# minaskar/tempest

Measured on AMD Instinct MI355X. Metric: particle-mutation-steps/s (whole job), 10-D Rosenbrock, higher is better.
Workload: dtype f64; 1 GPU; rosenbrock10d_n1048576 (BASELINE config 4: 10-D Rosenbrock, 1048576 particles sharded over 1 GPU(s), 1048576 per GPU); n_dim=10, particles_per_gpu=1048576, particles_global=1048576, sample=tpcn, resample=mult, clustering=False, n_total=4194304, step=one PS iteration, callbacks=torch-ROCm tensor callbacks (the drop-in contract: prior20, rosenbrock_torch)

## Files before the change

include/tempest_hip.h:

```cpp
#ifndef TEMPEST_HIP_H
#define TEMPEST_HIP_H

#include <stdint.h>

#ifdef __cplusplus
extern "C" {
#endif

typedef struct tph_ctx tph_ctx;

#define TPH_VERSION 100

#define TPH_KERNEL_TPCN 0
#define TPH_KERNEL_RWM 1

#define TPH_BC_STRICT 0
#define TPH_BC_PERIODIC 1
#define TPH_BC_REFLECTIVE 2

#define TPH_KEY_U 0
#define TPH_KEY_X 1
#define TPH_KEY_LOGL 2
#define TPH_KEY_LOGMIX 3

// ... 27 lines not shown
#define TPH_OPT_MF_DEAL 19
#define TPH_OPT_BLK_STAGE 20
#define TPH_OPT_GMM_KERNEL 21
#define TPH_OPT_FORMS_MFMA 22
int tph_set_option(tph_ctx* ctx, int option, int value);

typedef int (*tph_allreduce_fn)(void* user, int64_t offset, int64_t count, int dtype, int op);
typedef int (*tph_allgather_fn)(void* user, int64_t send_offset, int64_t recv_offset, int64_t count, int dtype);
int tph_comm_attach(tph_ctx* ctx, int rank, int world, void* buf_dev, int64_t buf_bytes, tph_allreduce_fn allreduce,
                    tph_allgather_fn allgather, void* user);
int tph_comm_detach(tph_ctx* ctx);
#define TPH_P2P_HANDLE_BYTES 64
int tph_comm_p2p_export(tph_ctx* ctx, void* handle_out );
int tph_comm_p2p_attach(tph_ctx* ctx, const void* handles , int* ok_out);
int tph_comm_p2p_active(const tph_ctx* ctx);
int tph_comm_p2p_status(tph_ctx* ctx);
int tph_comm_stats(tph_ctx* ctx, int64_t* out , int reset);
int tph_comm_allreduce_dev(tph_ctx* ctx, void* data_dev, int64_t count, int dtype, int op);

int tph_history_append(tph_ctx* ctx, const double* u_dev, const double* x_dev, const double* logl_dev,
                       int64_t n, int64_t ld, double beta, double logz, int64_t n_global);
int64_t tph_history_size(const tph_ctx* ctx);
int tph_history_iterations(const tph_ctx* ctx);
int tph_history_clear(tph_ctx* ctx);
int tph_history_memory(tph_ctx* ctx, int64_t* out9_host);
int tph_history_read(tph_ctx* ctx, int key, int64_t off, int64_t n, double* out_host);
int tph_history_ptr(tph_ctx* ctx, int key, void** dev_ptr, int64_t* ld);
int tph_history_load(tph_ctx* ctx, const double* u_host, const double* x_host, const double* logl_host,
                     int64_t n, int T, const double* beta_t, const double* logz_t, const int64_t* n_t_local,
                     const int64_t* n_t_global);

int tph_reweight_partials(tph_ctx* ctx, const double* betas_host, int nb, double* out_dev );
int tph_reweight_eval(tph_ctx* ctx, const double* betas_host, int nb, double* out_host );
int tph_weights(tph_ctx* ctx, double beta, double vmax, double s1, double* w_dev);
int tph_logw(tph_ctx* ctx, double beta, int64_t n_h_global, double* logw_dev);

int tph_trim_threshold_global(tph_ctx* ctx, const double* w_dev, int64_t n, double ess, int bins,
                              double* out_dev , double* out_host );
int tph_cdf_global(tph_ctx* ctx, const double* w_dev, int64_t n, const double* thr_dev , double* cdf_dev,
                   double* total_host );
int tph_resample_select_global(tph_ctx* ctx, const double* cdf_dev, int64_t n, int64_t n_slots, int scheme, uint64_t seed,
                               uint32_t tick, uint32_t tag, double u0, double pscale, int64_t* idx_dev);
int tph_resample_put_global(tph_ctx* ctx, const int64_t* idx_dev , int64_t n_slots, int64_t n_local,
                            double* u_out, double* x_out, double* logl_out, int64_t ld_out);
int tph_multinomial_counts_global(tph_ctx* ctx, const double* cdf_dev, int64_t n, const double* kept_count_dev, int factor,
                                  int64_t n_draw_max, uint64_t seed, uint32_t tick, uint32_t tag, int32_t* counts_dev);
int tph_fit_modes_global(tph_ctx* ctx, const int32_t* counts_dev, const int32_t* labels_dev, int64_t n, int K,
                         double* means_dev, double* covs_dev, double* chol_dev, double* inv_dev, double* cholinv_dev );

int tph_sum_sq_max(tph_ctx* ctx, const double* w_dev, int64_t n, double* out_host );

int tph_trim_threshold(tph_ctx* ctx, const double* w_dev, int64_t n, double ess, int bins,
                       double* out_dev , double* out_host );

int tph_cdf(tph_ctx* ctx, const double* w_dev, int64_t n, const double* thr_dev , double* cdf_dev);
int tph_resample_systematic(tph_ctx* ctx, const double* cdf_dev, int64_t n, int64_t n_out, int64_t i0,
                            int64_t size_global, double u0, double renorm, int64_t* idx_dev);
int tph_resample_multinomial(tph_ctx* ctx, const double* cdf_dev, int64_t n, int64_t n_out, uint64_t seed,
                             uint32_t tick, uint32_t tag, int64_t item0, int64_t* idx_dev);
int tph_resample_select(tph_ctx* ctx, const double* cdf_dev, int64_t n, int64_t n_slots, int scheme, uint64_t seed,
                        uint32_t tick, uint32_t tag, double u0, double w_before, double w_upto, double w_total,
                        int is_last, int64_t* idx_dev);
int tph_gather(tph_ctx* ctx, const int64_t* idx_dev, int64_t n_out, double* u_out, double* x_out,
               double* logl_out, int64_t ld_out);
int tph_posterior_rows(tph_ctx* ctx, int key, const int64_t* idx_dev, int64_t m, const double* w_dev, double wdiv,
                       double* x_out , double* logl_out , double* w_out );
// ... 91 lines not shown
```

tempest_amd/_lib.py:

```python
import ctypes as C
import os

_HERE = os.path.dirname(os.path.abspath(__file__))
LIB_PATH = os.path.join(_HERE, "csrc", "libtempest_hip.so")

c_i64 = C.c_int64
c_u64 = C.c_uint64
c_u32 = C.c_uint32
c_dbl = C.c_double
c_int = C.c_int
ptr = C.c_void_p

SIGNATURES = {
    "tph_last_error": (C.c_char_p, []),
    "tph_version": (c_int, []),
    "tph_ctx_create": (c_int, [c_int, c_int, c_i64, ptr, C.POINTER(ptr)]),
    "tph_ctx_destroy": (c_int, [ptr]),
    "tph_set_stream": (c_int, [ptr, ptr]),
    "tph_synchronize": (c_int, [ptr]),
    "tph_warmup": (c_int, [ptr]),
    "tph_set_option": (c_int, [ptr, c_int, c_int]),
    "tph_history_append": (c_int, [ptr, ptr, ptr, ptr, c_i64, c_i64, c_dbl, c_dbl, c_i64]),
    "tph_history_size": (c_i64, [ptr]),
    "tph_history_iterations": (c_int, [ptr]),
    "tph_history_clear": (c_int, [ptr]),
    "tph_history_memory": (c_int, [ptr, ptr]),
    "tph_history_read": (c_int, [ptr, c_int, c_i64, c_i64, ptr]),
    "tph_history_ptr": (c_int, [ptr, c_int, C.POINTER(ptr), C.POINTER(c_i64)]),
    "tph_history_load": (c_int, [ptr, ptr, ptr, ptr, c_i64, c_int, ptr, ptr, ptr, ptr]),
    "tph_reweight_partials": (c_int, [ptr, ptr, c_int, ptr]),
    "tph_reweight_eval": (c_int, [ptr, ptr, c_int, ptr]),
    "tph_bench_reweight_time": (c_int, [ptr, c_dbl, c_int, c_int, ptr]),
    "tph_bench_membw_time": (c_int, [ptr, c_int, c_i64, c_int, ptr]),
    "tph_bench_fp64_time": (c_int, [ptr, c_int, ptr]),
    "tph_student_sums": (c_int, [ptr, ptr, ptr, ptr, c_int, c_i64, ptr, c_int, ptr]),
    "tph_student_weights": (c_int, [ptr, ptr, ptr, ptr, c_int, c_i64, c_dbl, ptr]),
    "tph_bench_mf_normals": (c_int, [ptr, c_u64, c_u64, c_u64, c_int, ptr]),
    "tph_bench_mf_counters": (c_int, [ptr, ptr]),
    "tph_weights": (c_int, [ptr, c_dbl, c_dbl, c_dbl, ptr]),
    "tph_logw": (c_int, [ptr, c_dbl, c_i64, ptr]),
    "tph_sum_sq_max": (c_int, [ptr, ptr, c_i64, ptr]),
    "tph_trim_threshold": (c_int, [ptr, ptr, c_i64, c_dbl, c_int, ptr, ptr]),
    "tph_cdf": (c_int, [ptr, ptr, c_i64, ptr, ptr]),
    "tph_resample_systematic": (c_int, [ptr, ptr, c_i64, c_i64, c_i64, c_i64, c_dbl, c_dbl, ptr]),
    "tph_resample_multinomial": (c_int, [ptr, ptr, c_i64, c_i64, c_u64, c_u32, c_u32, c_i64, ptr]),
    "tph_resample_select": (c_int, [ptr, ptr, c_i64, c_i64, c_int, c_u64, c_u32, c_u32, c_dbl, c_dbl, c_dbl, c_dbl, c_int, ptr]),
    "tph_gather": (c_int, [ptr, ptr, c_i64, ptr, ptr, ptr, c_i64]),
    "tph_multinomial_counts": (c_int, [ptr, ptr, c_i64, ptr, c_int, c_i64, c_u64, c_u32, c_u32, ptr]),
    "tph_prior_draw": (c_int, [ptr, ptr, c_i64, c_i64, c_u64, c_u32, c_i64]),
    "tph_inf_repair": (c_int, [ptr, ptr, ptr, ptr, c_i64, c_i64, c_u64, c_u32, c_i64, ptr]),
    "tph_inf_repair_src": (c_int, [ptr, ptr, ptr, ptr, c_i64, c_i64, c_u64, c_u32, c_i64, ptr, ptr]),
    "tph_propose": (c_int, [ptr, c_int, ptr, ptr, c_i64, c_i64, c_int, ptr, ptr, ptr, ptr, ptr, ptr,
                            c_u64, c_u32, c_i64, ptr, ptr, ptr, ptr, ptr]),
    "tph_accept": (c_int, [ptr, c_int, c_dbl, ptr, ptr, ptr, ptr, ptr, ptr, ptr, ptr, ptr, c_i64, c_i64,
                           c_int, ptr, c_u64, c_u32, c_i64, ptr, ptr, ptr, ptr]),
    "tph_adapt": (c_int, [ptr, c_int, ptr, ptr, c_int, c_dbl, c_int, c_int, c_int, ptr, ptr, ptr, c_int, ptr, c_i64]),
    "tph_accept_sums_global": (c_int, [ptr, ptr, c_i64, c_int, ptr, c_int]),
    "tph_posterior_rows": (c_int, [ptr, c_int, ptr, c_i64, ptr, c_dbl, ptr, ptr, ptr]),
    "tph_marginals_layout": (c_i64, [c_int]),
    "tph_marginals_scratch_words": (c_i64, [c_i64, c_int, c_int, c_int, c_int, c_int]),
    "tph_marginals": (c_int, [ptr, ptr, c_i64, c_int, ptr, ptr, c_int, ptr, c_int, c_int, ptr, c_int, ptr, ptr, c_i64,
                              ptr, ptr, ptr, ptr, ptr, ptr, ptr, ptr]),
    "tph_index_compose": (c_int, [ptr, ptr, ptr, c_i64, ptr]),
    "tph_cluster_counts": (c_int, [ptr, ptr, c_i64, c_int, ptr]),
# ... 2 lines not shown
    "tph_weighted_moments": (c_int, [ptr, ptr, c_i64, ptr]),
    "tph_weighted_sums": (c_int, [ptr, ptr, c_i64, ptr]),
    "tph_weighted_cov_centered": (c_int, [ptr, ptr, c_i64, ptr, ptr]),
    "tph_weighted_moments_shifted": (c_int, [ptr, ptr, c_i64, ptr, ptr]),
    "tph_compact_indices": (c_int, [ptr, ptr, c_i64, ptr, ptr]),
    "tph_gather_u_affine": (c_int, [ptr, ptr, c_i64, ptr, ptr, ptr, ptr, c_i64, ptr]),
    "tph_affine": (c_int, [ptr, ptr, c_i64, c_i64, ptr, ptr]),
    "tph_x_weighted_sums": (c_int, [ptr, ptr, c_i64, c_i64, ptr, ptr, ptr]),
    "tph_x_weighted_cov": (c_int, [ptr, ptr, c_i64, c_i64, ptr, ptr, ptr]),
    "tph_gmm_estep": (c_int, [ptr, ptr, c_i64, c_i64, ptr, ptr, c_int, c_int, ptr, c_int, c_dbl, ptr, ptr, ptr, ptr, ptr]),
    "tph_gmm_em_state_doubles": (c_i64, [c_int, c_int]),
    "tph_gmm_em_begin": (c_int, [ptr, ptr, c_i64, c_i64, c_int, ptr, ptr]),
    "tph_gmm_em_run": (c_int, [ptr, ptr, c_i64, c_i64, ptr, ptr, c_int, c_int, ptr, ptr, c_dbl, c_dbl, c_int, c_int]),
    "tph_cv_sum": (c_int, [ptr, ptr, c_i64, ptr, ptr, ptr]),
    "tph_volume_variation": (c_int, [ptr, ptr, c_i64, ptr, ptr]),
    "tph_comm_attach": (c_int, [ptr, c_int, c_int, ptr, c_i64, ptr, ptr, ptr]),
    "tph_comm_detach": (c_int, [ptr]),
    "tph_comm_p2p_export": (c_int, [ptr, ptr]),
    "tph_comm_p2p_attach": (c_int, [ptr, ptr, ptr]),
    "tph_comm_p2p_active": (c_int, [ptr]),
    "tph_comm_p2p_status": (c_int, [ptr]),
    "tph_comm_stats": (c_int, [ptr, ptr, c_int]),
    "tph_comm_allreduce_dev": (c_int, [ptr, ptr, c_i64, c_int, c_int]),
    "tph_resample_put_global": (c_int, [ptr, ptr, c_i64, c_i64, ptr, ptr, ptr, c_i64]),
    "tph_trim_threshold_global": (c_int, [ptr, ptr, c_i64, c_dbl, c_int, ptr, ptr]),
    "tph_cdf_global": (c_int, [ptr, ptr, c_i64, ptr, ptr, ptr]),
    "tph_resample_select_global": (c_int, [ptr, ptr, c_i64, c_i64, c_int, c_u64, c_u32, c_u32, c_dbl, c_dbl, ptr]),
    "tph_multinomial_counts_global": (c_int, [ptr, ptr, c_i64, ptr, c_int, c_i64, c_u64, c_u32, c_u32, ptr]),
    "tph_fit_modes_global": (c_int, [ptr, ptr, ptr, c_i64, c_int, ptr, ptr, ptr, ptr, ptr]),
}

ALLREDUCE_FN = C.CFUNCTYPE(c_int, ptr, c_i64, c_i64, c_int, c_int)
ALLGATHER_FN = C.CFUNCTYPE(c_int, ptr, c_i64, c_i64, c_i64, c_int)


class TempestHipError(RuntimeError):
    pass


_lib = None


def load(path=None):
    global _lib
    if _lib is not None and path is None:
        return _lib
    p = path or LIB_PATH
    import torch
    if not os.path.exists(p):
        raise TempestHipError(
            f"{p} not found: the HIP extension is not built (run `make -C tempest_amd/csrc`). "
            "tempest_amd has no CPU fallback.")
    lib = C.CDLL(p)
    missing = []
    for name, (res, args) in SIGNATURES.items():
        try:
            fn = getattr(lib, name)
        except AttributeError:
            missing.append(name)
            continue
        fn.restype = res
        fn.argtypes = args
    if missing:
        raise TempestHipError(f"{p} lacks symbols declared in include/tempest_hip.h: {missing}")
    _lib = lib
    return lib
# ... 7 lines not shown
```

tempest_amd/csrc/resample.hip:

```cpp
#include "common.h"
#include "scan.h"
#include "cdf_index.h"
#include <cstring>
#include <rocprim/rocprim.hpp>

int tph_cdf_plain(tph_ctx* ctx, const double* w_dev, int64_t n, const double* thr_dev, double* cdf_dev) {
  if (tph_scratch_reserve(ctx, sizeof(double) * (size_t)tph_scan::num_tiles(n))) return -1;
  double* tiles = (double*)ctx->scratch;
  return thr_dev ? tph_scan::inclusive<tph_scan::MASKED>(ctx, w_dev, n, thr_dev, tiles, cdf_dev)
                 : tph_scan::inclusive<tph_scan::PLAIN>(ctx, w_dev, n, nullptr, tiles, cdf_dev);
}
static int cdf_pieces(tph_ctx* ctx, const double* w_dev, const double* thr_dev, double* cdf_dev, const tph_part& part);
extern "C" int tph_cdf(tph_ctx* ctx, const double* w_dev, int64_t n, const double* thr_dev, double* cdf_dev) {
  TPH_REQUIRE(ctx && w_dev && cdf_dev && n > 0, "tph_cdf: bad argument");
  const bool internal = ctx->scratch && (const char*)w_dev >= (const char*)ctx->scratch && (const char*)w_dev < (const char*)ctx->scratch + ctx->scratch_bytes;
  if (!ctx->comm_active() && !internal) {
    const tph_part part = tph_partition(ctx, n);
    if (part.canonical) return cdf_pieces(ctx, w_dev, thr_dev, cdf_dev, part);
  }
  if (tph_scratch_reserve(ctx, sizeof(double) * (size_t)tph_scan::num_tiles(n))) return -1;
  double* tiles = (double*)ctx->scratch;
  return thr_dev ? tph_scan::inclusive<tph_scan::MASKED>(ctx, w_dev, n, thr_dev, tiles, cdf_dev)
                 : tph_scan::inclusive<tph_scan::PLAIN>(ctx, w_dev, n, nullptr, tiles, cdf_dev);
}
// ... 312 lines not shown
  hipLaunchKernelGGL(k_select_global, dim3((unsigned)((n_slots + 255) / 256)), dim3(256), 0, ctx->stream, ix, ctx->blk_table,
                     ctx->blk_T, ctx->blk_rows, ctx->rank, ctx->world, n_slots, scheme, seed, tick, tag, u0, pscale, idx_dev);
  TPH_LAUNCH_CHECK();
  return 0;
}

__global__ void __launch_bounds__(256) k_counts_global(tph_cdf_index ix, const double* __restrict__ table, int T, int64_t rows,
                                                       int rank, int world, const double* __restrict__ kept_count_dev, int factor,
                                                       int64_t n_draw_max, uint64_t seed, uint32_t tick, uint32_t tag,
                                                       int32_t* __restrict__ counts) {
  int64_t n_draw = kept_count_dev ? (int64_t)(kept_count_dev[0]) * factor : n_draw_max;
  if (n_draw > n_draw_max) n_draw = n_draw_max;
  for (int64_t r = (int64_t)blockIdx.x * blockDim.x + threadIdx.x; r < n_draw; r += (int64_t)gridDim.x * blockDim.x) {
    tph_rng g(seed, tick, tag, (uint64_t)r);
    double U, U1;
    g.uniform2(0, U, U1);
    const double p = U * table[2 * T];
    const int t = owner_block<true>(table, T, rank, world, p);
    if (t < 0) continue;
    int64_t k = tph_count_below<false>(ix, 1.0, p);
    const int64_t first = (int64_t)t * rows, last = first + rows - 1;
    k = k < first ? first : (k > last ? last : k);
    atomicAdd(&counts[k], 1);
  }
}

extern "C" int tph_multinomial_counts_global(tph_ctx* ctx, const double* cdf_dev, int64_t n, const double* kept_count_dev,
                                             int factor, int64_t n_draw_max, uint64_t seed, uint32_t tick, uint32_t tag,
                                             int32_t* counts_dev) {
  TPH_REQUIRE(ctx && cdf_dev && counts_dev && n > 0 && n_draw_max > 0, "tph_multinomial_counts_global: bad argument");
  if (!ctx->comm_active())
    return tph_multinomial_counts(ctx, cdf_dev, n, kept_count_dev, factor, n_draw_max, seed, tick, tag, counts_dev);
  TPH_REQUIRE(ctx->blk_T > 0 && (int64_t)ctx->blk_T * ctx->blk_rows == n, "tph_multinomial_counts_global: call tph_cdf_global on this history first");
  TPH_HIP(hipMemsetAsync(counts_dev, 0, sizeof(int32_t) * (size_t)n, ctx->stream));
  TPH_HIP(hipMemsetAsync(counts_dev, 0, sizeof(int32_t) * (size_t)n, ctx->stream));
  if (tph_scratch_reserve(ctx, sizeof(double) * tph_cdf_index_doubles(n))) return -1;
  tph_cdf_index ix;
  if (tph_cdf_index_build(ctx, cdf_dev, n, (double*)ctx->scratch, &ix)) return -1;
  int64_t blocks = (n_draw_max + 255) / 256;
  if (blocks > 16 * (int64_t)ctx->n_simd) blocks = 16 * (int64_t)ctx->n_simd;
  hipLaunchKernelGGL(k_counts_global, dim3((unsigned)blocks), dim3(256), 0, ctx->stream, ix, ctx->blk_table,
                     ctx->blk_T, ctx->blk_rows, ctx->rank, ctx->world, kept_count_dev, factor, n_draw_max, seed, tick, tag, counts_dev);
  TPH_LAUNCH_CHECK();
  return 0;
}

constexpr int ROWS_TILE = 64;
__global__ void __launch_bounds__(256) k_rows_pack(const double* __restrict__ hu, const double* __restrict__ hx,
                                                   const double* __restrict__ hl, int64_t cap, int d, int64_t off, int64_t n,
                                                   double* __restrict__ rows) {
  extern __shared__ double tile[];
  const int rec = 2 * d + 1, pitch = rec + 1;
  const int64_t i0 = off + (int64_t)blockIdx.x * ROWS_TILE;
  const int64_t end = off + n;
  for (int e = threadIdx.x; e < ROWS_TILE * rec; e += 256) {
    const int c = e / ROWS_TILE, r = e - c * ROWS_TILE;
    const int64_t i = i0 + r;
    if (i < end) tile[r * pitch + c] = c < d ? hu[(size_t)c * cap + i] : (c < 2 * d ? hx[(size_t)(c - d) * cap + i] : hl[i]);
  }
  __syncthreads();
  for (int e = threadIdx.x; e < ROWS_TILE * rec; e += 256) {
    const int r = e / rec, c = e - r * rec;
    if (i0 + r < end) rows[(size_t)(i0 + r) * rec + c] = tile[r * pitch + c];
  }
}

void tph_rows_drop(tph_ctx* ctx) {
// ... 379 lines not shown
```

tempest_amd/csrc/reweight.hip:

```cpp
#include "common.h"

struct tph_betas { double b[TPH_MAX_NB]; };

struct trip { double m, s1, s2; };

__device__ __forceinline__ double2 nt_load2(const double2* p) {
  typedef double v2d __attribute__((ext_vector_type(2)));
  v2d a = __builtin_nontemporal_load(reinterpret_cast<const v2d*>(p));
  return make_double2(a.x, a.y);
}

__device__ __forceinline__ trip trip_merge(trip a, trip b) {
  double M = fmax(a.m, b.m);
  double fa = exp(a.m - M), fb = exp(b.m - M);
  trip r;
  r.m = M;
  r.s1 = a.s1 * fa + b.s1 * fb;
  r.s2 = a.s2 * (fa * fa) + b.s2 * (fb * fb);
  return r;
}

__device__ __forceinline__ trip trip_wave_reduce(trip t) {
#pragma unroll
  for (int o = 32; o > 0; o >>= 1) {
    trip b;
    b.m = __shfl_down(t.m, o, 64);
    b.s1 = __shfl_down(t.s1, o, 64);
    b.s2 = __shfl_down(t.s2, o, 64);
    t = trip_merge(t, b);
  }
  return t;
}

// ... 223 lines not shown
}

static int reweight_pass(tph_ctx* ctx, const tph_betas& bt, int nb, double* out, double* seq_host, double seq) {
  const tph_part part = tph_partition(ctx, ctx->size);
  const k2_geom g = k2_geometry(ctx, part);
  if (tph_partials_reserve(ctx, sizeof(double) * 3 * (size_t)nb * g.vl * g.bv)) return -1;
  launch_reduce_nb(ctx, g, bt, nb);
  TPH_LAUNCH_CHECK();
  if (ctx->comm_active()) {
    const size_t mine = 0, one = sizeof(double) * 3 * (size_t)nb * g.vl, all = (one + 255) / 256 * 256;
    if (tph_comm_require(ctx, all + one * ctx->world, "tph_reweight (sharded)")) return -2;
    hipLaunchKernelGGL(k_reweight_vshards, dim3(g.vl), dim3(1024), 0, ctx->stream, ctx->partials, g.bv, nb, (double*)(ctx->comm_buf + mine));
    TPH_LAUNCH_CHECK();
    if (tph_comm_allgather(ctx, mine, all, 3 * (int64_t)nb * g.vl, TPH_DT_F64)) return -2;
    hipLaunchKernelGGL(k_reweight_fold, dim3(nb), dim3(64), 0, ctx->stream, (const double*)nullptr, 0, (const double*)(ctx->comm_buf + all),
                       g.vl * ctx->world, nb, out, seq_host, seq, (unsigned int*)(ctx->small_dev + 4096));
  } else {
    hipLaunchKernelGGL(k_reweight_fold, dim3(nb), dim3(1024), 0, ctx->stream, (const double*)ctx->partials, g.bv, (const double*)nullptr, g.vl, nb,
                       out, seq_host, seq, (unsigned int*)(ctx->small_dev + 4096));
  }
  TPH_LAUNCH_CHECK();
  return 0;
}

extern "C" int tph_reweight_partials(tph_ctx* ctx, const double* betas_host, int nb, double* out_dev) {
  TPH_REQUIRE(ctx && betas_host && out_dev, "tph_reweight_partials: NULL argument");
  TPH_REQUIRE(nb >= 1 && nb <= TPH_MAX_NB, "tph_reweight_partials: nb=%d outside [1,%d]", nb, TPH_MAX_NB);
  TPH_REQUIRE(ctx->size > 0, "tph_reweight_partials: empty history");
  tph_betas bt;
  for (int i = 0; i < TPH_MAX_NB; ++i) bt.b[i] = i < nb ? betas_host[i] : 0.0;
  return reweight_pass(ctx, bt, nb, out_dev, nullptr, 0.0);
}

extern "C" int tph_reweight_eval(tph_ctx* ctx, const double* betas_host, int nb, double* out_host) {
  TPH_REQUIRE(ctx && betas_host && out_host, "tph_reweight_eval: NULL argument");
  TPH_REQUIRE(nb >= 1 && nb <= TPH_MAX_NB, "tph_reweight_eval: nb=%d outside [1,%d]", nb, TPH_MAX_NB);
  TPH_REQUIRE(ctx->size > 0, "tph_reweight_eval: empty history");
  tph_betas bt;
  for (int i = 0; i < TPH_MAX_NB; ++i) bt.b[i] = i < nb ? betas_host[i] : 0.0;
  volatile double* seqp = ctx->pinned + 4095;
  const double seq = (double)(++ctx->eval_seq);
  const int rc = reweight_pass(ctx, bt, nb, ctx->pinned, ctx->pinned + 4095, seq);
  if (rc) return rc;
  uint64_t spins = 0;
  while (*seqp != seq) {
    __builtin_ia32_pause();
    if ((++spins & 0xFFFFF) == 0) {
      hipError_t q = hipStreamQuery(ctx->stream);
      if (q != hipErrorNotReady) {
        TPH_HIP(hipStreamSynchronize(ctx->stream));
        TPH_REQUIRE(*seqp == seq, "tph_reweight_eval: the device never delivered evaluation %.0f", seq);
      }
    }
  }
  __atomic_thread_fence(__ATOMIC_ACQUIRE);
  for (int i = 0; i < 3 * nb; ++i) out_host[i] = ctx->pinned[i];
  return 0;
}

extern "C" int tph_bench_reweight_time(tph_ctx* ctx, double beta, int nb, int reps, double* avg_ms_host) {
  TPH_REQUIRE(ctx && avg_ms_host && reps > 0, "tph_bench_reweight_time: bad argument");
  TPH_REQUIRE(nb >= 1 && nb <= TPH_MAX_NB && ctx->size > 0, "tph_bench_reweight_time: bad nb / empty history");
  tph_betas bt;
  for (int i = 0; i < TPH_MAX_NB; ++i) bt.b[i] = beta * (1.0 - 0.01 * i);
  const k2_geom g = k2_geometry(ctx, tph_partition(ctx, ctx->size));
  if (tph_partials_reserve(ctx, sizeof(double) * 3 * (size_t)nb * g.vl * g.bv)) return -1;
  hipEvent_t e0, e1;
  TPH_HIP(hipEventCreate(&e0));
  TPH_HIP(hipEventCreate(&e1));
  launch_reduce_nb(ctx, g, bt, nb);
  TPH_HIP(hipEventRecord(e0, ctx->stream));
  for (int r = 0; r < reps; ++r) launch_reduce_nb(ctx, g, bt, nb);
  TPH_HIP(hipEventRecord(e1, ctx->stream));
  TPH_HIP(hipEventSynchronize(e1));
  float ms = 0.f;
  TPH_HIP(hipEventElapsedTime(&ms, e0, e1));
  TPH_HIP(hipEventDestroy(e0));
  TPH_HIP(hipEventDestroy(e1));
  *avg_ms_host = (double)ms / reps;
  return 0;
}

template <int MODE>
__global__ void __launch_bounds__(TPH_RED_THREADS) k_membw(const double* __restrict__ src, double* __restrict__ dst, int64_t n,
                                                          double* __restrict__ sink) {
  constexpr int U = 8;
  const int64_t n2 = n >> 1;
  const double2* __restrict__ s2 = reinterpret_cast<const double2*>(src);
  typedef double v2d __attribute__((ext_vector_type(2)));
  v2d* __restrict__ d2 = reinterpret_cast<v2d*>(dst);
// ... 158 lines not shown
```

tempest_amd/device.py:

```python
import ctypes as C

import numpy as np
import torch

from . import _lib
from ._lib import check

KERNEL_ID = {"tpcn": 0, "rwm": 1}
KEY_U, KEY_X, KEY_LOGL, KEY_LOGMIX = 0, 1, 2, 3
STEP_STATE_LEN = 10
OPT_ML_UNSTAGED = 3
OPT_BLOCKED = 4
OPT_MODES_EPOCH = 5
OPT_ROW_MIRROR = 6
OPT_COV_KERNEL = 7
OPT_SORTED_DRAWS = 8
OPT_STAGED_REDRAW = 9
OPT_SM_LANES = 10
OPT_SM_THRESHOLD = 11
OPT_SCREEN = 12
OPT_MF_LANES = 13
OPT_MF_AUDIT = 14
OPT_BLK_MFMA = 15
OPT_BLK_TRIES = 16
# ... 1 lines not shown
OPT_HISTORY_VM = 18
OPT_MF_DEAL = 19
OPT_BLK_STAGE = 20
OPT_GMM_KERNEL = 21
OPT_FORMS_MFMA = 22
BC_STRICT, BC_PERIODIC, BC_REFLECTIVE = 0, 1, 2

TAG_PRIOR, TAG_NORMAL, TAG_GAMMA, TAG_ACCEPT, TAG_RESAMPLE, TAG_UPSAMPLE, TAG_REPAIR, TAG_SYST = 1, 2, 3, 4, 5, 6, 7, 8


def _ptr(t, dtype=None):
    if t is None:
        return None
    if not t.is_cuda:
        raise _lib.TempestHipError("expected a device tensor")
    if dtype is not None and t.dtype != dtype:
        raise _lib.TempestHipError(f"expected dtype {dtype}, got {t.dtype}")
    if not t.is_contiguous():
        raise _lib.TempestHipError("expected a contiguous tensor")
    return t.data_ptr()


def vshards_for(n_global: int) -> int:
    for v in (48, 16, 12, 8, 6, 4, 3, 2, 1):
        if n_global > 0 and n_global % (v * 256) == 0:
            return v
    return 1


def _hptr(a):
    return a.ctypes.data_as(C.c_void_p)


class HipContext:

    def __init__(self, n_dim, device=None, capacity_hint=0):
        self.lib = _lib.load()
        if not torch.cuda.is_available():
            raise _lib.TempestHipError("no GPU visible: tempest_amd has no CPU fallback")
        if device is None:
            device = torch.cuda.current_device()
        self.device = torch.device("cuda", device if isinstance(device, int) else torch.device(device).index or 0)
        self.n_dim = int(n_dim)
        torch.cuda.set_device(self.device)
        self._ctx = C.c_void_p()
        self.rows_hint = int(capacity_hint)
        stream = torch.cuda.current_stream(self.device).cuda_stream
        check(self.lib.tph_ctx_create(self.device.index, self.n_dim, int(capacity_hint), C.c_void_p(stream),
                                      C.byref(self._ctx)), "tph_ctx_create")

    def close(self):
        if getattr(self, "_ctx", None) is not None and self._ctx:
            self.lib.tph_ctx_destroy(self._ctx)
            self._ctx = None

    def __del__(self):
        try:
            self.close()
        except Exception:
            pass

    def empty(self, *shape, dtype=torch.float64):
        return torch.empty(*shape, dtype=dtype, device=self.device)

    def empty_rows(self, n, dtype=torch.float64):
        n = int(n)
# ... 56 lines not shown
    def history_load(self, u, x, logl, beta_t, logz_t, n_t, n_t_global=None, soa=False):
        logl = np.ascontiguousarray(logl, dtype=np.float64)
        n = logl.size
        self._vv_centre = None
        tr = (lambda a: a) if soa else (lambda a: a.T)
        ut = np.ascontiguousarray(tr(np.asarray(u, dtype=np.float64))) if u is not None else None
        xt = np.ascontiguousarray(tr(np.asarray(x, dtype=np.float64))) if x is not None else None
        for a in (ut, xt):
            if a is not None and a.shape != (self.n_dim, n):
                raise _lib.TempestHipError(f"history_load: array of shape {a.shape}, expected {(self.n_dim, n)}")
        bt = np.ascontiguousarray(beta_t, dtype=np.float64)
        zt = np.ascontiguousarray(logz_t, dtype=np.float64)
        nt = np.ascontiguousarray(n_t, dtype=np.int64)
        ng = np.ascontiguousarray(n_t if n_t_global is None else n_t_global, dtype=np.int64)
        check(self.lib.tph_history_load(self._ctx, _hptr(ut) if ut is not None else None,
                                        _hptr(xt) if xt is not None else None, _hptr(logl), n, bt.size,
                                        _hptr(bt), _hptr(zt), _hptr(nt), _hptr(ng)), "tph_history_load")

    def history_read(self, key, off=0, n=None, soa=False):
        n = self.size - off if n is None else n
        if key in (KEY_U, KEY_X):
            buf = np.empty((self.n_dim, n), dtype=np.float64)
        else:
            buf = np.empty((n,), dtype=np.float64)
        if n > 0:
            check(self.lib.tph_history_read(self._ctx, key, off, n, _hptr(buf)), "tph_history_read")
        return np.ascontiguousarray(buf.T) if (buf.ndim == 2 and not soa) else buf

    def reweight_eval(self, betas):
        b = np.ascontiguousarray(np.atleast_1d(betas), dtype=np.float64)
        out = np.empty((b.size, 3), dtype=np.float64)
        check(self.lib.tph_reweight_eval(self._ctx, _hptr(b), b.size, _hptr(out)), "tph_reweight_eval")
        return out

    def reweight_partials(self, betas, out=None):
        b = np.ascontiguousarray(np.atleast_1d(betas), dtype=np.float64)
        if out is None:
            out = self.empty(b.size, 3)
        check(self.lib.tph_reweight_partials(self._ctx, _hptr(b), b.size, _ptr(out, torch.float64)),
              "tph_reweight_partials")
        return out

    def reweight_time(self, beta=0.37, nb=1, reps=20):
        out = C.c_double(0.0)
        check(self.lib.tph_bench_reweight_time(self._ctx, float(beta), int(nb), int(reps), C.byref(out)), "tph_bench_reweight_time")
        return out.value

    P2P_HANDLE_BYTES = 64

    def p2p_export(self) -> bytes:
        h = C.create_string_buffer(self.P2P_HANDLE_BYTES)
        check(self.lib.tph_comm_p2p_export(self._ctx, h), "tph_comm_p2p_export")
        return h.raw

    def p2p_attach(self, handles) -> bool:
        blob = b"".join(handles)
        ok = C.c_int(0)
        check(self.lib.tph_comm_p2p_attach(self._ctx, C.c_char_p(blob), C.byref(ok)), "tph_comm_p2p_attach")
        return bool(ok.value)

    @property
    def p2p_active(self) -> bool:
        return bool(self.lib.tph_comm_p2p_active(self._ctx))

    def comm_stats(self, reset=False):
        out = (C.c_int64 * 5)()
# ... 371 lines not shown
```

tempest_amd/state_manager.py:

```python
import os
from pathlib import Path
from typing import Optional, Union

import numpy as np

CURRENT_STATE_KEYS = frozenset({
    "u", "x", "logl", "assignments", "blobs", "acceptance", "steps", "efficiency", "ess", "cv", "beta", "logz",
    "calls", "iter",
})
HISTORY_STATE_KEYS = frozenset({
    "u", "x", "logl", "blobs", "iter", "logz", "calls", "steps", "efficiency", "ess", "cv", "acceptance", "beta",
})
REQUIRED_COMMIT_KEYS = frozenset({"beta", "logl"})

_DEVICE_ARRAYS = ("u", "x", "logl")
_SCALAR_HISTORY = tuple(sorted(HISTORY_STATE_KEYS - set(_DEVICE_ARRAYS) - {"blobs"}))


class StateManager:

    def __init__(self, n_dim: int, device=None, comm=None, capacity_hint: int = 0):
        self.n_dim = n_dim
        self._device_arg = device
        self._capacity_hint = capacity_hint
# ... 156 lines not shown
        if logl is not None:
            import torch
            beta, logz = self._current["beta"], self._current["logz"]
            if beta is None:
                raise ValueError("cannot commit particle arrays without 'beta' (it defines the mixture term)")
            n = int(logl.shape[0])
            u, x = self._current["u"], self._current["x"]
            if u is None:
                u = torch.zeros(self.n_dim, n, dtype=torch.float64, device=self.device)
            if x is None:
                x = torch.zeros(self.n_dim, n, dtype=torch.float64, device=self.device)
            n_glob = n if self.comm is None else n * self.comm.world_size
            self.ctx.use_current_stream()
            self.ctx.history_append(u.contiguous(), x.contiguous(), logl.contiguous(), float(beta),
                                    0.0 if logz is None else float(logz), n_glob)
            self._n_local.append(n)
            self._n_global.append(n_glob)
        for k in _SCALAR_HISTORY:
            v = self._current[k]
            if v is not None:
                self._scalars[k].append(v.copy() if isinstance(v, np.ndarray) else v)
        if self._current["blobs"] is not None:
            self._blobs.append(np.array(self._current["blobs"], copy=True))
        self._invalidate_cache()

    def n_history_global(self) -> int:
        return int(np.sum(self._n_global)) if self._n_global else 0

    def reweight_eval(self, betas):
        ctx = self.ctx
        ctx.use_current_stream()
        return ctx.reweight_eval(betas)

    def compute_logw_and_logz(self, beta_final: float = 1.0, normalize: bool = True):
        if self.get_history_length() == 0 or len(self._n_local) == 0:
            return np.array([]), -np.inf
        if len(self._n_local) != self.get_history_length():
            raise ValueError("history of 'beta' and of the particle arrays differ in length")
        m, s1, _ = self.reweight_eval([beta_final])[0]
        logz = float(m + np.log(s1))
        nh = self.n_history_global()
        logw = self.ctx.logw(beta_final, nh).cpu().numpy()
        if normalize:
            logw = logw - (logz + np.log(nh))
        return logw, logz

    def compute_results(self) -> dict:
        if self._results_dict is None:
            out = {}
            for key in HISTORY_STATE_KEYS:
                if key == "blobs" and not self._blobs:
                    out[key] = np.array([])
                    continue
                out[key] = self.get_history(key)
            out["logw"], _ = self.compute_logw_and_logz(1.0)
            self._results_dict = out
        return self._results_dict

    def to_dict(self) -> dict:
        hist = {k: list(v) for k, v in self._scalars.items()}
        for key in _DEVICE_ARRAYS:
            hist[key] = [self.get_history(key, index=t) for t in range(len(self._n_local))]
        hist["blobs"] = list(self._blobs)
        return {"_current": self.get_current(), "_history": hist, "n_dim": self.n_dim}

    @classmethod
# ... 67 lines not shown
```

tempest_amd/steps/reweight.py:

```python
import math
from typing import Optional

import numpy as np


class DeviceWeights:

    def __init__(self, dev, beta=None, triple=None):
        self.dev = dev
        self.beta = beta
        self.triple = triple

    def __len__(self):
        return int(self.dev.numel())

    @property
    def shape(self):
        return (len(self),)

    def __array__(self, dtype=None, copy=None):
        a = self.dev.cpu().numpy()
        return a.astype(dtype) if dtype is not None else a


class Reweighter:

    _MAX_BISECTION_ITERATIONS = 200

    def __init__(self, state, pbar=None, n_particles: int = 256, ess_ratio: float = 2.0,
                 volume_variation: Optional[float] = None, ESS_TOLERANCE: float = 0.001,
                 BETA_TOLERANCE: float = 1e-5, BETA_RTOL: float = 1e-8, METRIC_ATOL: float = 0.5,
                 METRIC_ATOL_CV: float = 0.01):
        self.state = state
        self.pbar = pbar
        self.n_particles = n_particles
        self.ess_ratio = ess_ratio
        self.volume_variation = volume_variation
        self.target_metric = volume_variation if volume_variation is not None else ess_ratio * n_particles
        self.ESS_TOLERANCE = ESS_TOLERANCE
        self.BETA_TOLERANCE = BETA_TOLERANCE
        self.BETA_RTOL = BETA_RTOL
        self.METRIC_ATOL = METRIC_ATOL
        self.METRIC_ATOL_CV = METRIC_ATOL_CV
        self.n_evals = 0
        self.n_passes = 0
        self.batch_depth = None
        self._cache = {}

    def _eval_many(self, betas):
        todo = []
        for b in betas:
            if b not in self._cache and b not in todo:
                todo.append(b)
        for i in range(0, len(todo), 16):
            chunk = todo[i:i + 16]
            res = self.state.reweight_eval(chunk)
            self.n_passes += 1
            for b, (m, s1, s2) in zip(chunk, res):
                self._cache[b] = (float(m), float(s1), float(s2), float(s1 * s1 / s2))
                self.n_evals += 1

    def _eval(self, beta: float):
        hit = self._cache.get(beta)
        if hit is None:
            self._eval_many([beta])
            hit = self._cache[beta]
        return hit

    @staticmethod
    def _midpoint_tree(lo: float, hi: float, depth: int):
        out, level = [], [(lo, hi)]
        for _ in range(depth):
            nxt = []
            for a, b in level:
                mid = (b + a) * 0.5
                out.append(mid)
                nxt.append((a, mid))
                nxt.append((mid, b))
            level = nxt
        return out

    def _depth(self) -> int:
        if self.batch_depth is not None:
            return self.batch_depth
        rows = max(1, self.state.ctx.size)
        best, best_cost = 1, None
        for k in (1, 2, 3, 4):
            cost = (90.0 + max(rows * 4e-6, rows * 2.2e-6 * (2 ** k - 1))) / k
            if best_cost is None or cost < best_cost:
                best, best_cost = k, cost
        return best

    def _prefetch(self, lo: float, hi: float, extra=()):
        mid = (hi + lo) * 0.5
        bd = self._depth()
        if bd > 1 and mid not in self._cache:
            depth = bd if not extra else min(bd, 3)
            self._eval_many(list(extra) + self._midpoint_tree(lo, hi, depth))

    def _weights_dev(self, beta: float):
# ... 52 lines not shown
        if self._depth() > 1:
            self._prefetch(beta_low, beta_high, extra=(beta_current, 1.0))
        if self._eval(beta_current)[3] <= ess_target:
            return beta_current, beta_current
        if self._eval(1.0)[3] >= ess_target:
            return 1.0, 1.0
        while True:
            beta_mid = (beta_high + beta_low) * 0.5
            if (beta_high - beta_low) <= self._tol(beta_low, beta_high):
                break
            self._prefetch(beta_low, beta_high)
            if self._eval(beta_mid)[3] >= ess_target:
                beta_low = beta_mid
            else:
                beta_high = beta_mid
        return beta_low, beta_high

    def run(self):
        st = self.state
        self._cache = {}
        it = st.get_current("iter") + 1
        st.set_current("iter", it)
        if self.pbar is not None:
            self.pbar.update_iter()

        if st.get_history_length() == 0:
            st.update_current({"beta": 0.0, "logz": 0.0, "ess": self.ess_ratio * self.n_particles, "cv": 0.0})
            if self.pbar is not None:
                self.pbar.update_stats(dict(beta=0.0, ESS=int(self.ess_ratio * self.n_particles), logZ=0.0, CV=0.0))
            return np.broadcast_to(np.float64(1.0 / self.n_particles), (self.n_particles,))

        beta_prev = st.get_current("beta")
        ess_target = self.ess_ratio * self.n_particles
        beta_low, beta_high = self._find_ess_bracket(beta_prev, ess_target)

        if self.volume_variation is None:
            if beta_low == beta_high:
                beta = beta_low
            else:
                beta, _ = self._find_beta_bisection(beta_prev, beta_high, ess_target,
                                                    lambda b: (self._eval(b)[3], None))
        else:
            if beta_low == beta_high:
                beta = beta_low
            else:
                vv_prev, vv_high = self._cv(beta_prev), self._cv(beta_high)
                if self.volume_variation >= vv_high:
                    beta = beta_high
                elif self.volume_variation <= vv_prev:
                    beta = beta_prev
                else:
                    beta, _ = self._find_beta_bisection(beta_prev, beta_high, self.volume_variation,
                                                        lambda b: (self._cv(b), None))
        m, s1, _, ess = self._eval(beta)
        w = self._weights_dev(beta)
        from ..tools import device_volume_variation
        cv = device_volume_variation(st.ctx, w, st.n_history_global(), st.comm)
        logz = m + math.log(s1)
        if self.pbar is not None:
            self.pbar.update_stats(dict(beta=beta, ESS=int(ess), logZ=logz, CV=cv))
        st.update_current({"logz": logz, "beta": beta, "ess": ess, "cv": cv})
        return DeviceWeights(w, beta, (m, s1))
```

Measured before the change: 2.098 billion particle-mutation-steps/s.

## Move ESS beta bracket and bisection search into native C++ loop

Adds a C++ beta search that runs the ESS bracket and bisection loop natively. It uses a depth-tuned midpoint prefetch tree and memoises results, so each search step no longer makes a Python round trip. The Python reweight step now calls this native search whenever no volume-variation target or custom batch depth is set. A duplicated memset in the global multinomial counts path is also removed. Risks are behavioural drift from the Python search and hard-coded cost-model constants that pick the prefetch depth.

After: 1.510 billion particle-mutation-steps/s. 28.0% lower.

```diff
diff --git a/include/tempest_hip.h b/include/tempest_hip.h
--- a/include/tempest_hip.h
+++ b/include/tempest_hip.h
@@ -83,6 +83,13 @@
 
 int tph_reweight_partials(tph_ctx* ctx, const double* betas_host, int nb, double* out_dev );
 int tph_reweight_eval(tph_ctx* ctx, const double* betas_host, int nb, double* out_host );
+typedef int (*tph_beta_eval_fn)(void* user, const double* betas, int nb, double* out );
+int tph_reweight_search(tph_ctx* ctx, double beta_prev, double ess_target, double ess_tolerance, double beta_tolerance,
+                        double beta_rtol, double metric_atol, int depth, double* out8_host, int32_t* counts3_host,
+                        double* asked_host, int asked_cap);
+int tph_beta_search_fn(tph_beta_eval_fn eval, void* user, int64_t rows, double beta_prev, double ess_target,
+                       double ess_tolerance, double beta_tolerance, double beta_rtol, double metric_atol, int depth,
+                       double* out8_host, int32_t* counts3_host, double* asked_host, int asked_cap);
 int tph_weights(tph_ctx* ctx, double beta, double vmax, double s1, double* w_dev);
 int tph_logw(tph_ctx* ctx, double beta, int64_t n_h_global, double* logw_dev);
 
diff --git a/tempest_amd/_lib.py b/tempest_amd/_lib.py
--- a/tempest_amd/_lib.py
+++ b/tempest_amd/_lib.py
@@ -30,6 +30,8 @@
     "tph_history_load": (c_int, [ptr, ptr, ptr, ptr, c_i64, c_int, ptr, ptr, ptr, ptr]),
     "tph_reweight_partials": (c_int, [ptr, ptr, c_int, ptr]),
     "tph_reweight_eval": (c_int, [ptr, ptr, c_int, ptr]),
+    "tph_reweight_search": (c_int, [ptr, c_dbl, c_dbl, c_dbl, c_dbl, c_dbl, c_dbl, c_int, ptr, ptr, ptr, c_int]),
+    "tph_beta_search_fn": (c_int, [ptr, ptr, c_i64, c_dbl, c_dbl, c_dbl, c_dbl, c_dbl, c_dbl, c_int, ptr, ptr, ptr, c_int]),
     "tph_bench_reweight_time": (c_int, [ptr, c_dbl, c_int, c_int, ptr]),
     "tph_bench_membw_time": (c_int, [ptr, c_int, c_i64, c_int, ptr]),
     "tph_bench_fp64_time": (c_int, [ptr, c_int, ptr]),
@@ -98,6 +100,7 @@
 
 ALLREDUCE_FN = C.CFUNCTYPE(c_int, ptr, c_i64, c_i64, c_int, c_int)
 ALLGATHER_FN = C.CFUNCTYPE(c_int, ptr, c_i64, c_i64, c_i64, c_int)
+BETA_EVAL_FN = C.CFUNCTYPE(c_int, ptr, C.POINTER(c_dbl), c_int, C.POINTER(c_dbl))
 
 
 class TempestHipError(RuntimeError):
diff --git a/tempest_amd/csrc/beta_search.h b/tempest_amd/csrc/beta_search.h
--- /dev/null
+++ b/tempest_amd/csrc/beta_search.h
@@ -0,0 +1,169 @@
+#pragma once
+#include <cmath>
+#include <cfloat>
+#include <cstdint>
+#include <vector>
+
+#include "../../include/tempest_hip.h"
+
+constexpr int TPH_BS_MAX_BISECTIONS = 200;
+constexpr int TPH_BS_MAX_DEPTH = 4;
+constexpr int TPH_BS_PASS_BETAS = 16;
+
+constexpr double TPH_BS_PASS_FIXED_US = 15.0;
+constexpr double TPH_BS_PASS_FIXED_COMM_US = 90.0;
+constexpr double TPH_BS_ROW_FLOOR_US = 3.0e-6;
+constexpr double TPH_BS_CU_ROW_BETA_US = 4.15e-4;
+constexpr double TPH_BS_CUS = 256.0;
+static inline int tph_bs_depth(double rows, double block_rows, double fixed_us) {
+#pragma clang fp contract(off)
+  if (rows < 1.0) rows = 1.0;
+  if (block_rows < 1.0) block_rows = 1.0;
+  const double cu_rows = rows / TPH_BS_CUS > block_rows ? rows / TPH_BS_CUS : block_rows;
+  int best = 1;
+  double best_cost = 0.0;
+  for (int k = 1; k <= TPH_BS_MAX_DEPTH; ++k) {
+    const double work = cu_rows * TPH_BS_CU_ROW_BETA_US * (double)((1 << k) - 1), floor_us = rows * TPH_BS_ROW_FLOOR_US;
+    const double cost = (fixed_us + (work > floor_us ? work : floor_us)) / (double)k;
+    if (k == 1 || cost < best_cost) { best = k; best_cost = cost; }
+  }
+  return best;
+}
+
+struct tph_bs_entry { double beta, m, s1, s2, ess; };
+
+struct tph_bs_result {
+  double beta, m, s1, s2, ess, beta_low, beta_high;
+  int depth, n_evals, n_passes;
+};
+
+struct tph_beta_search {
+  tph_beta_eval_fn eval;
+  void* user;
+  double ess_tolerance, beta_tolerance, beta_rtol, metric_atol;
+  int depth;
+  std::vector<tph_bs_entry> memo;
+  std::vector<double> asked;
+  int n_evals = 0, n_passes = 0, rc = 0;
+
+  const tph_bs_entry* find(double b) const {
+    for (const tph_bs_entry& e : memo)
+      if (e.beta == b) return &e;
+    return nullptr;
+  }
+
+  void eval_many(const double* betas, int n) {
+#pragma clang fp contract(off)
+    std::vector<double> todo;
+    for (int i = 0; i < n; ++i) {
+      bool known = find(betas[i]) != nullptr;
+      for (size_t j = 0; j < todo.size() && !known; ++j) known = todo[j] == betas[i];
+      if (!known) todo.push_back(betas[i]);
+    }
+    for (size_t i = 0; i < todo.size(); i += TPH_BS_PASS_BETAS) {
+      const int nb = (int)(todo.size() - i < (size_t)TPH_BS_PASS_BETAS ? todo.size() - i : (size_t)TPH_BS_PASS_BETAS);
+      double out[3 * TPH_BS_PASS_BETAS];
+      const int r = rc ? rc : eval(user, todo.data() + i, nb, out);
+      if (r && !rc) rc = r;
+      ++n_passes;
+      for (int b = 0; b < nb; ++b) {
+        tph_bs_entry e;
+        e.beta = todo[i + b];
+        if (r) { e.m = e.s1 = e.s2 = e.ess = NAN; }
+        else {
+          e.m = out[3 * b]; e.s1 = out[3 * b + 1]; e.s2 = out[3 * b + 2];
+          const double sq = e.s1 * e.s1;
+          e.ess = sq / e.s2;
+        }
+        memo.push_back(e);
+        ++n_evals;
+      }
+    }
+  }
+
+  tph_bs_entry at(double beta) {
+    bool seen = false;
+    for (size_t j = 0; j < asked.size() && !seen; ++j) seen = asked[j] == beta;
+    if (!seen) asked.push_back(beta);
+    const tph_bs_entry* hit = find(beta);
+    if (!hit) { eval_many(&beta, 1); hit = find(beta); }
+    return *hit;
+  }
+
+  void prefetch(double lo, double hi, bool ends, double end0, double end1) {
+#pragma clang fp contract(off)
+    const double mid = (hi + lo) * 0.5;
+    if (depth <= 1 || find(mid)) return;
+    const int levels = ends ? (depth < 3 ? depth : 3) : depth;
+    std::vector<double> betas;
+    if (ends) { betas.push_back(end0); betas.push_back(end1); }
+    std::vector<double> level{lo, hi}, next;
+    for (int l = 0; l < levels; ++l) {
+      next.clear();
+      for (size_t i = 0; i < level.size(); i += 2) {
+        const double a = level[i], b = level[i + 1], m = (b + a) * 0.5;
+        betas.push_back(m);
+        next.push_back(a); next.push_back(m);
+        next.push_back(m); next.push_back(b);
+      }
+      level.swap(next);
+    }
+    eval_many(betas.data(), (int)betas.size());
+  }
+
+  double tol(double lo, double hi) const {
+#pragma clang fp contract(off)
+    double scale = std::fabs(lo);
+    if (std::fabs(hi) > scale) scale = std::fabs(hi);
+    if (DBL_MIN > scale) scale = DBL_MIN;
+    const double a = beta_rtol * scale, b = beta_tolerance * scale;
+    return b > a ? b : a;
+  }
+
+  void bracket(double beta_current, double target, double* low, double* high) {
+#pragma clang fp contract(off)
+    double lo = beta_current, hi = 1.0;
+    if (depth > 1) prefetch(lo, hi, true, beta_current, 1.0);
+    if (at(beta_current).ess <= target) { *low = *high = beta_current; return; }
+    if (at(1.0).ess >= target) { *low = *high = 1.0; return; }
+    while (rc == 0) {
+      const double mid = (hi + lo) * 0.5;
+      if ((hi - lo) <= tol(lo, hi)) break;
+      prefetch(lo, hi, false, 0.0, 0.0);
+      if (at(mid).ess >= target) lo = mid;
+      else hi = mid;
+    }
+    *low = lo; *high = hi;
+  }
+
+  double bisect(double beta_min, double beta_max, double target) {
+#pragma clang fp contract(off)
+    double beta = beta_min;
+    for (int it = 0; it < TPH_BS_MAX_BISECTIONS && rc == 0; ++it) {
+      beta = (beta_max + beta_min) * 0.5;
+      prefetch(beta_min, beta_max, false, 0.0, 0.0);
+      double metric = at(beta).ess;
+      if (!std::isfinite(metric)) metric = 1e10;
+      const double rel = ess_tolerance * std::fabs(target);
+      const bool metric_converged = std::fabs(metric - target) < (metric_atol > rel ? metric_atol : rel);
+      const bool beta_converged = (beta_max - beta_min) < tol(beta_min, beta_max);
+      if (metric_converged || beta_converged || beta == 1.0) return beta;
+      if (metric < target) beta_max = beta;
+      else beta_min = beta;
+    }
+    return beta;
+  }
+
+  int run(double beta_prev, double target, tph_bs_result* res) {
+    double low, high;
+    bracket(beta_prev, target, &low, &high);
+    const double beta = (low == high || rc) ? low : bisect(beta_prev, high, target);
+    if (rc) return rc;
+    const tph_bs_entry e = at(beta);
+    if (rc) return rc;
+    res->beta = beta; res->m = e.m; res->s1 = e.s1; res->s2 = e.s2; res->ess = e.ess;
+    res->beta_low = low; res->beta_high = high;
+    res->depth = depth; res->n_evals = n_evals; res->n_passes = n_passes;
+    return 0;
+  }
+};
diff --git a/tempest_amd/csrc/resample.hip b/tempest_amd/csrc/resample.hip
--- a/tempest_amd/csrc/resample.hip
+++ b/tempest_amd/csrc/resample.hip
@@ -368,7 +368,6 @@
   if (!ctx->comm_active())
     return tph_multinomial_counts(ctx, cdf_dev, n, kept_count_dev, factor, n_draw_max, seed, tick, tag, counts_dev);
   TPH_REQUIRE(ctx->blk_T > 0 && (int64_t)ctx->blk_T * ctx->blk_rows == n, "tph_multinomial_counts_global: call tph_cdf_global on this history first");
-  TPH_HIP(hipMemsetAsync(counts_dev, 0, sizeof(int32_t) * (size_t)n, ctx->stream));
   TPH_HIP(hipMemsetAsync(counts_dev, 0, sizeof(int32_t) * (size_t)n, ctx->stream));
   if (tph_scratch_reserve(ctx, sizeof(double) * tph_cdf_index_doubles(n))) return -1;
   tph_cdf_index ix;
diff --git a/tempest_amd/csrc/reweight.hip b/tempest_amd/csrc/reweight.hip
--- a/tempest_amd/csrc/reweight.hip
+++ b/tempest_amd/csrc/reweight.hip
@@ -1,4 +1,5 @@
 #include "common.h"
+#include "beta_search.h"
 
 struct tph_betas { double b[TPH_MAX_NB]; };
 
@@ -288,10 +289,7 @@
   return reweight_pass(ctx, bt, nb, out_dev, nullptr, 0.0);
 }
 
-extern "C" int tph_reweight_eval(tph_ctx* ctx, const double* betas_host, int nb, double* out_host) {
-  TPH_REQUIRE(ctx && betas_host && out_host, "tph_reweight_eval: NULL argument");
-  TPH_REQUIRE(nb >= 1 && nb <= TPH_MAX_NB, "tph_reweight_eval: nb=%d outside [1,%d]", nb, TPH_MAX_NB);
-  TPH_REQUIRE(ctx->size > 0, "tph_reweight_eval: empty history");
+static int reweight_eval_host(tph_ctx* ctx, const double* betas_host, int nb, double* out_host) {
   tph_betas bt;
   for (int i = 0; i < TPH_MAX_NB; ++i) bt.b[i] = i < nb ? betas_host[i] : 0.0;
   volatile double* seqp = ctx->pinned + 4095;
@@ -312,6 +310,67 @@
   __atomic_thread_fence(__ATOMIC_ACQUIRE);
   for (int i = 0; i < 3 * nb; ++i) out_host[i] = ctx->pinned[i];
   return 0;
+}
+
+extern "C" int tph_reweight_eval(tph_ctx* ctx, const double* betas_host, int nb, double* out_host) {
+  TPH_REQUIRE(ctx && betas_host && out_host, "tph_reweight_eval: NULL argument");
+  TPH_REQUIRE(nb >= 1 && nb <= TPH_MAX_NB, "tph_reweight_eval: nb=%d outside [1,%d]", nb, TPH_MAX_NB);
+  TPH_REQUIRE(ctx->size > 0, "tph_reweight_eval: empty history");
+  return reweight_eval_host(ctx, betas_host, nb, out_host);
+}
+
+static int bs_copy_out(const tph_beta_search& s, const tph_bs_result& r, double* out8, int32_t* counts3, double* asked, int asked_cap) {
+  out8[0] = r.beta; out8[1] = r.m; out8[2] = r.s1; out8[3] = r.s2; out8[4] = r.ess; out8[5] = r.beta_low; out8[6] = r.beta_high;
+  out8[7] = (double)r.depth;
+  counts3[0] = r.n_evals; counts3[1] = r.n_passes; counts3[2] = (int32_t)s.asked.size();
+  for (size_t i = 0; i < s.asked.size() && (int)i < asked_cap; ++i) asked[i] = s.asked[i];
+  return 0;
+}
+
+static int bs_check(const char* who, double beta_prev, double ess_target, int depth, const double* out8, const int32_t* counts3,
+                    const double* asked, int asked_cap) {
+  TPH_REQUIRE(out8 && counts3 && (asked || asked_cap == 0) && asked_cap >= 0, "%s: NULL output argument", who);
+  TPH_REQUIRE(depth >= 0 && depth <= TPH_BS_MAX_DEPTH, "%s: depth=%d outside [0,%d]", who, depth, TPH_BS_MAX_DEPTH);
+  TPH_REQUIRE(std::isfinite(beta_prev) && ess_target == ess_target, "%s: beta_prev=%g not finite, or the target is NaN", who, beta_prev);
+  return 0;
+}
+
+extern "C" int tph_beta_search_fn(tph_beta_eval_fn eval, void* user, int64_t rows, double beta_prev, double ess_target,
+                                  double ess_tolerance, double beta_tolerance, double beta_rtol, double metric_atol, int depth,
+                                  double* out8, int32_t* counts3, double* asked, int asked_cap) {
+  TPH_REQUIRE(eval, "tph_beta_search_fn: NULL evaluator");
+  if (int rc = bs_check("tph_beta_search_fn", beta_prev, ess_target, depth, out8, counts3, asked, asked_cap)) return rc;
+  const double nr = (double)(rows > 1 ? rows : 1);
+  tph_beta_search s{eval, user, ess_tolerance, beta_tolerance, beta_rtol, metric_atol,
+                    depth > 0 ? depth : tph_bs_depth(nr, nr < 16384.0 ? nr : 16384.0, TPH_BS_PASS_FIXED_US)};
+  tph_bs_result r;
+  if (int rc = s.run(beta_prev, ess_target, &r)) {
+    tph_set_error("tph_beta_search_fn: the evaluator failed (%d) after %d passes", rc, s.n_passes);
+    return rc;
+  }
+  return bs_copy_out(s, r, out8, counts3, asked, asked_cap);
+}
+
+static int bs_device_eval(void* user, const double* betas, int nb, double* out) {
+  return reweight_eval_host((tph_ctx*)user, betas, nb, out);
+}
+
+extern "C" int tph_reweight_search(tph_ctx* ctx, double beta_prev, double ess_target, double ess_tolerance, double beta_tolerance,
+                                   double beta_rtol, double metric_atol, int depth, double* out8, int32_t* counts3, double* asked,
+                                   int asked_cap) {
+  TPH_REQUIRE(ctx, "tph_reweight_search: NULL argument");
+  TPH_REQUIRE(ctx->size > 0, "tph_reweight_search: empty history");
+  if (int rc = bs_check("tph_reweight_search", beta_prev, ess_target, depth, out8, counts3, asked, asked_cap)) return rc;
+  if (depth == 0) {
+    const k2_geom g = k2_geometry(ctx, tph_partition(ctx, ctx->size));
+    const double blocks = (double)g.vl * (double)g.bv;
+    depth = tph_bs_depth((double)ctx->size, (double)ctx->size / (blocks > 1.0 ? blocks : 1.0),
+                         ctx->comm_active() ? TPH_BS_PASS_FIXED_COMM_US : TPH_BS_PASS_FIXED_US);
+  }
+  tph_beta_search s{bs_device_eval, ctx, ess_tolerance, beta_tolerance, beta_rtol, metric_atol, depth};
+  tph_bs_result r;
+  if (int rc = s.run(beta_prev, ess_target, &r)) return rc;
+  return bs_copy_out(s, r, out8, counts3, asked, asked_cap);
 }
 
 extern "C" int tph_bench_reweight_time(tph_ctx* ctx, double beta, int nb, int reps, double* avg_ms_host) {
diff --git a/tempest_amd/device.py b/tempest_amd/device.py
--- a/tempest_amd/device.py
+++ b/tempest_amd/device.py
@@ -57,6 +57,28 @@
     return a.ctypes.data_as(C.c_void_p)
 
 
+def unpack_search(out, counts, asked):
+    return {"beta": float(out[0]), "triple": (float(out[1]), float(out[2]), float(out[3])), "ess": float(out[4]),
+            "beta_low": float(out[5]), "beta_high": float(out[6]), "depth": int(out[7]), "n_evals": int(counts[0]),
+            "n_passes": int(counts[1]), "asked": [float(b) for b in asked[:min(int(counts[2]), asked.size)]]}
+
+
+def beta_search_fn(evaluate, rows, beta_prev, ess_target, ess_tolerance, beta_tolerance, beta_rtol, metric_atol, depth=0):
+    def cb(_user, betas, nb, res):
+        try:
+            for i, t in enumerate(evaluate([betas[j] for j in range(nb)])):
+                res[3 * i], res[3 * i + 1], res[3 * i + 2] = float(t[0]), float(t[1]), float(t[2])
+        except Exception:
+            return -3
+        return 0
+    fn = _lib.BETA_EVAL_FN(cb)
+    out, counts, asked = np.empty(8), np.zeros(3, dtype=np.int32), np.empty(2048)
+    check(_lib.load().tph_beta_search_fn(fn, None, int(rows), float(beta_prev), float(ess_target), float(ess_tolerance),
+                                         float(beta_tolerance), float(beta_rtol), float(metric_atol), int(depth),
+                                         _hptr(out), _hptr(counts), _hptr(asked), asked.size), "tph_beta_search_fn")
+    return unpack_search(out, counts, asked)
+
+
 class HipContext:
 
     def __init__(self, n_dim, device=None, capacity_hint=0):
@@ -179,6 +201,13 @@
         out = np.empty((b.size, 3), dtype=np.float64)
         check(self.lib.tph_reweight_eval(self._ctx, _hptr(b), b.size, _hptr(out)), "tph_reweight_eval")
         return out
+
+    def reweight_search(self, beta_prev, ess_target, ess_tolerance, beta_tolerance, beta_rtol, metric_atol, depth=0):
+        out, counts, asked = np.empty(8), np.zeros(3, dtype=np.int32), np.empty(2048)
+        check(self.lib.tph_reweight_search(self._ctx, float(beta_prev), float(ess_target), float(ess_tolerance),
+                                           float(beta_tolerance), float(beta_rtol), float(metric_atol), int(depth),
+                                           _hptr(out), _hptr(counts), _hptr(asked), asked.size), "tph_reweight_search")
+        return unpack_search(out, counts, asked)
 
     def reweight_partials(self, betas, out=None):
         b = np.ascontiguousarray(np.atleast_1d(betas), dtype=np.float64)
diff --git a/tempest_amd/state_manager.py b/tempest_amd/state_manager.py
--- a/tempest_amd/state_manager.py
+++ b/tempest_amd/state_manager.py
@@ -212,6 +212,11 @@
         ctx.use_current_stream()
         return ctx.reweight_eval(betas)
 
+    def reweight_search(self, *args, **kw):
+        ctx = self.ctx
+        ctx.use_current_stream()
+        return ctx.reweight_search(*args, **kw)
+
     def compute_logw_and_logz(self, beta_final: float = 1.0, normalize: bool = True):
         if self.get_history_length() == 0 or len(self._n_local) == 0:
             return np.array([]), -np.inf
diff --git a/tempest_amd/steps/reweight.py b/tempest_amd/steps/reweight.py
--- a/tempest_amd/steps/reweight.py
+++ b/tempest_amd/steps/reweight.py
@@ -45,6 +45,7 @@
         self.n_evals = 0
         self.n_passes = 0
         self.batch_depth = None
+        self.asked = []
         self._cache = {}
 
     def _eval_many(self, betas):
@@ -66,6 +67,11 @@
             self._eval_many([beta])
             hit = self._cache[beta]
         return hit
+
+    def _native_search(self):
+        if self.volume_variation is not None or self.batch_depth is not None or "_eval" in self.__dict__:
+            return None
+        return getattr(self.state, "reweight_search", None)
 
     @staticmethod
     def _midpoint_tree(lo: float, hi: float, depth: int):
@@ -184,7 +190,17 @@
 
         beta_prev = st.get_current("beta")
         ess_target = self.ess_ratio * self.n_particles
-        beta_low, beta_high = self._find_ess_bracket(beta_prev, ess_target)
+        native = self._native_search()
+        if native is not None:
+            res = native(beta_prev, ess_target, self.ESS_TOLERANCE, self.BETA_TOLERANCE, self.BETA_RTOL, self.METRIC_ATOL, 0)
+            beta = res["beta"]
+            self._cache[beta] = (*res["triple"], res["ess"])
+            self.n_evals += res["n_evals"]
+            self.n_passes += res["n_passes"]
+            self.asked = res["asked"]
+            beta_low = beta_high = beta
+        else:
+            beta_low, beta_high = self._find_ess_bracket(beta_prev, ess_target)
 
         if self.volume_variation is None:
             if beta_low == beta_high:
```
